# csyxwei/FFWM

Measured on AMD Instinct MI355X. Metric: train img/s (128x128, full FFWM GAN step), higher is better.
Workload: dtype f32; 1 GPU; BASELINE configs[2]: full FFWM train step (netG+netD+flowNetF+flowNetB, all losses, 3x Adam), synthetic MultiPIE-shaped 128x128; batch_per_gpu=8, global_batch=8, parallelism=dp1, grad_buckets=10, bucket_MiB=64

## Files before the change

ffwm_amd/_lib.py:

```python
import ctypes
import os

_HERE = os.path.dirname(os.path.abspath(__file__))
LIB_PATH = os.path.join(_HERE, "lib", "libffwm_hip.so")

F32, F64 = 0, 1
ABI_VERSION = 5

_lib = None

_p = ctypes.c_void_p
_i64 = ctypes.c_int64
_i = ctypes.c_int

_SIGNATURES = {
    "ffwm_block_extractor_forward": [_p, _p, _p] + [_i64] * 6 + [_i, _i, _p],
    "ffwm_block_extractor_backward": [_p, _p, _p, _p, _p] + [_i64] * 6 + [_i, _i, _p],
    "ffwm_block_extractor_backward_strided": [_p, _p, _p, ctypes.POINTER(_i64), _p, _p] + [_i64] * 6 + [_i, _i, _p],
    "ffwm_local_attn_reshape_backward_strided": [_p, ctypes.POINTER(_i64), _p] + [_i64] * 3 + [_i, _i, _i, _p],
    "ffwm_resample2d_backward_strided": [_p, _p, _p, ctypes.POINTER(_i64), _p, _p] + [_i64] * 6 + [_i, _i, _i, _i, _p],
    "ffwm_bn_lrelu_forward": [_p] * 9 + [_i64] * 3 + [ctypes.c_double] * 3 + [_i, _p],
    "ffwm_bn_lrelu_backward": [_p] * 10 + [_i64] * 3 + [ctypes.c_double] + [_i, _p],
    "ffwm_bn_res_act_forward": [_p] * 11 + [_i64] * 3 + [ctypes.c_double] * 3 + [_i, _i, _p],
    "ffwm_bn_res_act_backward": [_p] * 11 + [_i64] * 3 + [ctypes.c_double] + [_i, _i, _p],
# ... 23 lines not shown
    "ffwm_sgd_step": [_p, _p, _p, _i64, _p, _p, _i, _p, _p, _i, ctypes.c_double, _i, _p],
    "ffwm_softmax_xent": [_p] * 8 + [_i64, _i64, _i, _p],
    "ffwm_softmax_xent_chunk": [],
    "ffwm_conv3x3_wgrad": [_p, _p, _p, _p] + [_i64] * 5 + [_i, _p],
    "ffwm_conv3x3_wgrad_block": [_p, _p, _p, _p] + [_i64] * 9 + [_i, _p],
    "ffwm_block_attention_forward": [_p, _p, _p, _p] + [_i64] * 6 + [_i, _i, _p],
    "ffwm_block_attention_backward": [_p, _p, _p, _p, _p, _p, _p] + [_i64] * 6 + [_i, _i, _p],
    "ffwm_local_attn_reshape_forward": [_p, _p] + [_i64] * 3 + [_i, _i, _p],
    "ffwm_local_attn_reshape_backward": [_p, _p] + [_i64] * 3 + [_i, _i, _i, _p],
    "ffwm_resample2d_forward": [_p, _p, _p] + [_i64] * 6 + [_i, _i, _i, _p],
    "ffwm_resample2d_backward": [_p, _p, _p, _p, _p] + [_i64] * 6 + [_i, _i, _i, _i, _p],
    "ffwm_warp_forward": [_p, _p, _p] + [_i64] * 6 + [_i, _i, _p],
    "ffwm_warp_backward": [_p, _p, _p, _p, _p] + [_i64] * 6 + [_i, _i, _p],
    "ffwm_warp_multi_forward": [_p, _i, _i, _i, _p],
    "ffwm_warp_multi_backward": [_p, _i, _i, _i, _p],
    "ffwm_spectral_norm_forward": [_p, _i, _i, ctypes.c_double, _i, _p],
    "ffwm_spectral_norm_backward": [_p, _i, _i, _p],
    "ffwm_guided_filter_forward": [_p, _p, _p, _p, _i64, _i64, _i64, _i, ctypes.c_double, _i, _p],
    "ffwm_affine_regularization": [_p, _p, _p, _p, _i64, _i64, _i64, _i, ctypes.c_double, _i, _p],
    "ffwm_correlation_colmax": [_p, _p, _p, _i64, _i64, _i64, _i, _p],
    "ffwm_correlation_colmax_split": [_p, _p, _p, _i64, _i64, _i64, _i, _p],
    "ffwm_sampling_correctness": [_p] * 9 + [_i64] * 6 + [ctypes.c_double, ctypes.c_double, _i, _p],
    "ffwm_landmark_loss": [_p, _p, ctypes.POINTER(_i64), ctypes.POINTER(_i64), ctypes.POINTER(ctypes.c_double), _i] + [_p] * 6
                          + [_i64, _i64, _i, _p],
    "ffwm_guided_filter_backward": [_p, _p, _p, _p, _p, _p, _i64, _i64, _i64, _i, _i, _p],
    "ffwm_guided_filter_forward_general": [_p, _p, _p, _p, _p, _i64, _i64, _i64, _i64, _i, ctypes.c_double, _i, _p],
    "ffwm_guided_filter_backward_general": [_p, _p, _p, _p, _p, _p, _p, _i64, _i64, _i64, _i64, _i, _i, _p],
    "ffwm_l1_multi": [_p, _i, _p, _p, _i, _i, _p],
    "ffwm_conv3x3_winograd_weights_multi": [_p, _i, _i, _p],
    "ffwm_conv3x3_wg_weights": [_p, _p, _i64, _i64, _i, _i, _p],
    "ffwm_conv3x3_wg_forward": [_p, _p, _p, _p, _p] + [_i64] * 5 + [_i, _p, _i, _p],
    "ffwm_conv3x3_wg_forward_tiled": [_p, _p, _p, _p, _p] + [_i64] * 5 + [_i, _p, _i, _i, _p],
    "ffwm_conv3x3_wg_tile": [_i64] * 5,
    "ffwm_mfm_tail_forward": [_p, _p, _p, _p] + [_i64] * 4 + [_i, _i, _p],
    "ffwm_identity_input": [_p, _p] + [_i64] * 4 + [_i, _i, _p],
    "ffwm_identity_input_backward": [_p, _p] + [_i64] * 4 + [_i, _i, _p],
    "ffwm_cosine_topk": [_p, _p, _p, _p] + [_i64] * 4 + [_p, _i64, _i, _p],
    "ffwm_face_batch": [_p] * 16 + [_i64] * 8 + [_i, _p],
    "ffwm_face_gallery": [_p, _p, _p] + [_i64] * 4 + [_p],
    "ffwm_identity_batch": [_p] * 8 + [_i64] * 5 + [_i, _i, _p],
    "ffwm_prof_enable": [_i],
    "ffwm_prof_collect": [],
    "ffwm_prof_get": [_i, ctypes.c_char_p, _i, ctypes.POINTER(_i64), ctypes.POINTER(ctypes.c_double),
                      ctypes.POINTER(ctypes.c_double)],
    "ffwm_prof_get_flops": [_i, ctypes.POINTER(ctypes.c_double)],
    "ffwm_prof_get_bound": [_i, ctypes.POINTER(ctypes.c_double)],
    "ffwm_prof_reset": [],
    "ffwm_set_option": [ctypes.c_char_p, _i],
    "ffwm_zero_fill": [_p, _i64, _p],
    "ffwm_abi_version": [],
}

EXPORTS = sorted(list(_SIGNATURES) + ["ffwm_last_error", "ffwm_conv3x3_winograd_workspace_bytes", "ffwm_conv3x3_winograd_splits",
                                      "ffwm_conv2d_forward_workspace", "ffwm_guided_filter_workspace_bytes",
                                      "ffwm_sampling_correctness_workspace_bytes", "ffwm_landmark_loss_workspace_bytes",
                                      "ffwm_cosine_topk_workspace_bytes", "ffwm_softmax_xent_workspace_bytes",
                                      "ffwm_conv3x3_wg_weights_bytes", "ffwm_conv3x3_wg_workspace_bytes"])


class FFWMError(RuntimeError):
    pass


def load():
    global _lib
    if _lib is not None:
        return _lib
    if not os.path.exists(LIB_PATH):
        raise FFWMError(
            "libffwm_hip.so is missing (%s). The HIP extension is the only implementation of the "
            "ffwm_amd ops -- build it with `python -m ffwm_amd.build`." % LIB_PATH)
    lib = ctypes.CDLL(LIB_PATH)
    for name, argtypes in _SIGNATURES.items():
        fn = getattr(lib, name)
        fn.argtypes = argtypes
        fn.restype = _i
    lib.ffwm_conv3x3_winograd_workspace_bytes.argtypes = [_i64, _i64]
    lib.ffwm_conv3x3_winograd_workspace_bytes.restype = _i64
    lib.ffwm_conv3x3_winograd_splits.argtypes = [_i64, _i64, _i64, _i64, _i64, _i]
    lib.ffwm_conv3x3_winograd_splits.restype = _i
    lib.ffwm_conv2d_forward_workspace.argtypes = [_i64] * 5 + [_i] * 4
    lib.ffwm_conv2d_forward_workspace.restype = _i64
    lib.ffwm_guided_filter_workspace_bytes.argtypes = [_i64] * 4 + [_i, _i]
    lib.ffwm_guided_filter_workspace_bytes.restype = _i64
    lib.ffwm_sampling_correctness_workspace_bytes.argtypes = [_i64, _i64, _i64, _i]
    lib.ffwm_sampling_correctness_workspace_bytes.restype = _i64
    lib.ffwm_landmark_loss_workspace_bytes.argtypes = [ctypes.POINTER(_i64), _i, _i64, _i64, _i]
    lib.ffwm_landmark_loss_workspace_bytes.restype = _i64
    lib.ffwm_softmax_xent_workspace_bytes.argtypes = [_i64, _i64, _i]
    lib.ffwm_softmax_xent_workspace_bytes.restype = _i64
    lib.ffwm_cosine_topk_workspace_bytes.argtypes = [_i64] * 4
    lib.ffwm_cosine_topk_workspace_bytes.restype = _i64
    lib.ffwm_conv3x3_wg_weights_bytes.argtypes = [_i64, _i64]
    lib.ffwm_conv3x3_wg_weights_bytes.restype = _i64
    lib.ffwm_conv3x3_wg_workspace_bytes.argtypes = [_i64] * 5
    lib.ffwm_conv3x3_wg_workspace_bytes.restype = _i64
    lib.ffwm_last_error.argtypes = []
    lib.ffwm_last_error.restype = ctypes.c_char_p
    got = lib.ffwm_abi_version()
    if got != ABI_VERSION:
        raise FFWMError("libffwm_hip.so ABI version %d, expected %d: rebuild it" % (got, ABI_VERSION))
    _lib = lib
    for kv in filter(None, os.environ.get("FFWM_OPTS", "").split(",")):
        k, _, v = kv.partition("=")
        if lib.ffwm_set_option(k.strip().encode(), int(v)) < 0:
            raise FFWMError("FFWM_OPTS: unknown option %r (or a negative value)" % k)
    return lib


def check(rc, what):
    if rc != 0:
        msg = load().ffwm_last_error()
        raise FFWMError("%s failed (status %d): %s" % (what, rc, msg.decode() if msg else "?"))


def prof_enable(on=True):
    return load().ffwm_prof_enable(1 if on else 0)


def prof_reset():
    load().ffwm_prof_reset()


def prof_collect():
    lib = load()
    n = lib.ffwm_prof_collect()
    rows = {}
    for i in range(n):
        name = ctypes.create_string_buffer(128)
# ... 22 lines not shown
```

ffwm_amd/conv.py:

```python
import os as _os

import torch
import torch.nn as nn
from torch.autograd import Function

from . import ops

_WGRAD_W64 = _os.environ.get("FFWM_WGRAD_W64", "1") == "1"


class _Conv3x3MfmaWgrad(Function):

    @staticmethod
    def forward(ctx, x, weight, bias):
        ctx.save_for_backward(x, weight)
        ctx.has_bias = bias is not None
        return torch.ops.aten.convolution(x, weight, bias, [1, 1], [1, 1], [1, 1], False, [0, 0], 1)

    @staticmethod
    @torch.autograd.function.once_differentiable
    def backward(ctx, grad_output):
        x, weight = ctx.saved_tensors
        go = grad_output.contiguous()
        need_x, need_w, need_b = ctx.needs_input_grad[0], ctx.needs_input_grad[1], ctx.has_bias and ctx.needs_input_grad[2]
# ... 77 lines not shown
        self.off = self.need = 0
        if self.buf is not None and self.buf.device != device:
            self.retired.append(self.buf)
            self.buf = None
        if self.buf is not None:
            ops.zero_fill(self.buf)
        self.active = True
        self.device = device

    def take(self, n, like):
        if not self.active or like.device != self.device or like.dtype != torch.float32:
            return None
        n_al = (n + 63) & ~63
        self.need += n_al
        if self.buf is None or self.off + n_al > self.buf.numel():
            return None
        s = self.buf[self.off:self.off + n]
        self.off += n_al
        return s

    def end(self):
        if not self.active:
            return
        self.active = False
        if (self.buf is None or self.need > self.buf.numel()) and self.need > 0 and not torch.cuda.is_current_stream_capturing():
            if self.buf is not None:
                self.retired.append(self.buf)
            self.buf = torch.zeros(self.need + self.need // 8, device=self.device, dtype=torch.float32)


GRAD_ARENA = _GradArena()


def conv_weight_grad(x, go, weight, stride, pad, need_b):
    k = weight.shape[2]
    if k == 3 and stride == 1 and pad == 1 and wgrad_route_ok(x, weight):
        n = weight.numel()
        total = n + (weight.shape[0] if need_b else 0)
        buf = GRAD_ARENA.take(total, go)
        if buf is None:
            buf = torch.zeros(total, device=go.device, dtype=go.dtype)
        gw, gb = buf[:n].view_as(weight), (buf[n:] if need_b else None)
        ops.conv3x3_wgrad(x, go, gw, gb)
        return gw, gb
    if _tiled_wgrad_wins(go, x, k) and weight.shape[2] == weight.shape[3]:
        return ops.conv2d_wgrad_tiled(go, x, k, stride, pad, want_bias=bool(need_b),
                                      zeroed=GRAD_ARENA.take(weight.numel() + (weight.shape[0] if need_b else 0), go))
    _, gw, gb = torch.ops.aten.convolution_backward(go, x, weight, [weight.shape[0]] if need_b else None, [stride, stride], [pad, pad],
                                                    [1, 1], False, [0, 0], 1, [False, True, bool(need_b)])
    return gw, gb


def conv_transpose_weight_grad(x, go, weight, need_b):
    if _tiled_wgrad_wins(x, go, 4):
        gw, _ = ops.conv2d_wgrad_tiled(x, go, 4, 2, 1, zeroed=GRAD_ARENA.take(weight.numel(), go))
        return gw, (_bias_grad(go) if need_b else None)
    _, gw, gb = torch.ops.aten.convolution_backward(go, x, weight, [weight.shape[1]] if need_b else None, [2, 2], [1, 1], [1, 1], True,
                                                    [0, 0], 1, [False, True, bool(need_b)])
    return gw, gb


_WINOGRAD = _os.environ.get("FFWM_WINOGRAD", "1") != "0"
WINOGRAD_MIN_TILES = int(_os.environ.get("FFWM_WINOGRAD_MIN_TILES", 2048))
WINOGRAD_MIN_PAIRS = int(_os.environ.get("FFWM_WINOGRAD_MIN_PAIRS", 160))


def _winograd_dir_ok(x, c_red, k_out, act=0):
    tiles = x.shape[0] * ((x.shape[2] + 1) // 2) * ((x.shape[3] + 1) // 2)
    if not (min(c_red, k_out) >= 32 and tiles >= WINOGRAD_MIN_TILES and x.shape[0] * max(c_red, k_out) * x.shape[2] * x.shape[3] < (1 << 29)):
        return False
    pairs = ((tiles + 63) // 64) * ((k_out + 63) // 64)
    if pairs < WINOGRAD_MIN_PAIRS and act == 0:
        pairs *= ops.conv3x3_winograd_splits(x.shape[0], c_red, x.shape[2], x.shape[3], k_out, act)
    return pairs >= WINOGRAD_MIN_PAIRS


def winograd_dirs(x, weight, act=0):
# ... 544 lines not shown
```

ffwm_amd/csrc/conv_winograd_gemm.hip:

```cpp
#include "common.hpp"

namespace ffwm {
namespace {

typedef float f32x16 __attribute__((ext_vector_type(16)));
typedef float f32x4 __attribute__((ext_vector_type(4)));

enum { kWgNone = FFWM_WG_NONE, kWgBias = FFWM_WG_BIAS, kWgBiasRelu = FFWM_WG_BIAS_RELU, kWgBiasMfm = FFWM_WG_BIAS_MFM };
constexpr int kWgStage = 16;

struct WgGeo {
    int C, C4;
    int H, W, K;
    int TH, TW, T;
    int Tp, Kp;
};

__device__ __forceinline__ float wg_max_nan(float a, float b) { return __builtin_isunordered(a, b) ? a + b : fmaxf(a, b); }
__device__ __forceinline__ float wg_relu_nan(float v) { return v != v ? v : fmaxf(v, 0.f); }

__global__ void __launch_bounds__(kBlock)
wg_weights_kernel(const float* __restrict__ w, float* __restrict__ U, int K, int C, int Cp, int mode) {
    const int64_t e = static_cast<int64_t>(blockIdx.x) * kBlock + threadIdx.x;
    if (e >= static_cast<int64_t>(K) * Cp) return;
// ... 49 lines not shown
        for (int i = 0; i < 4; ++i)
#pragma unroll
            for (int q = 0; q < 4; ++q) {
                const int iy = 2 * ty - 1 + i, ix = 2 * tx - 1 + q;
                float e = 0.f;
                if (cv && iy >= 0 && iy < g.H && ix >= 0 && ix < g.W) {
                    const size_t o = plane + static_cast<size_t>(iy) * g.W + ix;
                    e = x[o];
                    if (mask != nullptr) e = mask[o] <= 0.f ? 0.f : e;
                }
                d[i * 4 + q] = e;
            }
#pragma unroll
        for (int i = 0; i < 4; ++i) {
            float r[4];
#pragma unroll
            for (int q = 0; q < 4; ++q)
                r[q] = i == 0 ? d[0 + q] - d[8 + q] : i == 1 ? d[4 + q] + d[8 + q] : i == 2 ? d[8 + q] - d[4 + q] : d[4 + q] - d[12 + q];
            v[i * 4 + 0][j] = r[0] - r[2];
            v[i * 4 + 1][j] = r[1] + r[2];
            v[i * 4 + 2][j] = r[2] - r[1];
            v[i * 4 + 3][j] = r[1] - r[3];
        }
    }
    const size_t pstride = static_cast<size_t>(g.C4) * g.Tp;
    f32x4* dst = reinterpret_cast<f32x4*>(V) + static_cast<size_t>(c4) * g.Tp + t;
#pragma unroll
    for (int p = 0; p < 16; ++p) dst[p * pstride] = v[p];
}

template <int TILE>
__global__ void __launch_bounds__(kBlock)
wg_batched_gemm_kernel(const float* __restrict__ U, const float* __restrict__ V, float* __restrict__ M, int K, int C4, int Tp, int Kp,
                       int KT, int TTn) {
    constexpr int WT = TILE / 2, NB = WT / 32, NL = TILE / 64;
    __shared__ f32x4 As[2][4][TILE];
    __shared__ f32x4 Bs[2][4][TILE];
    const int lane = threadIdx.x & 63, wave = threadIdx.x >> 6;
    const int l31 = lane & 31, half = lane >> 5;
    const int wm = wave >> 1, wn = wave & 1;
    unsigned bid = blockIdx.x;
    const int tt = static_cast<int>(bid % static_cast<unsigned>(TTn));
    bid /= static_cast<unsigned>(TTn);
    const int kt = static_cast<int>(bid % static_cast<unsigned>(KT));
    const int p = static_cast<int>(bid / static_cast<unsigned>(KT));
    const int k0 = kt * TILE, t0 = tt * TILE;
    const f32x4* Up = reinterpret_cast<const f32x4*>(U) + static_cast<size_t>(p) * C4 * K;
    const f32x4* Vp = reinterpret_cast<const f32x4*>(V) + static_cast<size_t>(p) * C4 * Tp;

    f32x4 ra[NL], rb[NL];
    auto gload = [&](int stage) {
#pragma unroll
        for (int i = 0; i < NL; ++i) {
            const int idx = threadIdx.x + kBlock * i;
            const int grp = stage * 4 + idx / TILE, n = idx % TILE;
            f32x4 a = {0.f, 0.f, 0.f, 0.f};
            if (k0 + n < K) a = Up[static_cast<size_t>(grp) * K + k0 + n];
            ra[i] = a;
            rb[i] = Vp[static_cast<size_t>(grp) * Tp + t0 + n];
        }
    };
    auto sstore = [&](int buf) {
#pragma unroll
        for (int i = 0; i < NL; ++i) {
            const int idx = threadIdx.x + kBlock * i;
            As[buf][idx / TILE][idx % TILE] = ra[i];
            Bs[buf][idx / TILE][idx % TILE] = rb[i];
        }
    };

    f32x16 acc[NB][NB];
#pragma unroll
    for (int i = 0; i < NB; ++i)
#pragma unroll
        for (int j = 0; j < NB; ++j)
#pragma unroll
            for (int r = 0; r < 16; ++r) acc[i][j][r] = 0.f;

    const int stages = C4 / 4;
    gload(0);
    sstore(0);
    __syncthreads();
    int buf = 0;
    for (int st = 0; st < stages; ++st) {
        const bool more = st + 1 < stages;
        if (more) gload(st + 1);
#pragma unroll
        for (int s = 0; s < 2; ++s) {
            f32x4 a[NB], b[NB];
#pragma unroll
            for (int i = 0; i < NB; ++i) {
                a[i] = As[buf][2 * s + half][wm * WT + i * 32 + l31];
                b[i] = Bs[buf][2 * s + half][wn * WT + i * 32 + l31];
            }
#pragma unroll
            for (int q = 0; q < 4; ++q)
#pragma unroll
                for (int i = 0; i < NB; ++i)
#pragma unroll
                    for (int j = 0; j < NB; ++j)
                        acc[i][j] = __builtin_amdgcn_mfma_f32_32x32x2f32(a[i][q], b[j][q], acc[i][j], 0, 0, 0);
        }
        if (more) sstore(buf ^ 1);
        __syncthreads();
        buf ^= 1;
    }

    float* Mp = M + (static_cast<size_t>(p) * Kp + k0 + wm * WT) * Tp + t0 + wn * WT + l31;
#pragma unroll
    for (int i = 0; i < NB; ++i)
#pragma unroll
        for (int j = 0; j < NB; ++j)
#pragma unroll
            for (int r = 0; r < 16; ++r) {
                const int row = i * 32 + (r & 3) + 8 * (r >> 2) + 4 * half;
                Mp[static_cast<size_t>(row) * Tp + j * 32] = acc[i][j][r];
            }
}

__device__ __forceinline__ void wg_tile_of(const float* __restrict__ M, size_t pstride, float bv, float (&y)[4]) {
    float z[4][2];
#pragma unroll
    for (int i = 0; i < 4; ++i) {
        const float m0 = M[(i * 4 + 0) * pstride], m1 = M[(i * 4 + 1) * pstride], m2 = M[(i * 4 + 2) * pstride], m3 = M[(i * 4 + 3) * pstride];
        z[i][0] = (m0 + m1) + m2;
        z[i][1] = (m1 - m2) - m3;
    }
#pragma unroll
    for (int j = 0; j < 2; ++j) {
        y[j] = ((z[0][j] + z[1][j]) + z[2][j]) + bv;
        y[2 + j] = ((z[1][j] - z[2][j]) - z[3][j]) + bv;
    }
}

__global__ void __launch_bounds__(kBlock)
wg_output_transform_kernel(const float* __restrict__ M, const float* __restrict__ bias, float* __restrict__ out, const WgGeo g, int epi,
                           int vec) {
    const int t = blockIdx.x * kBlock + threadIdx.x;
    if (t >= g.T) return;
    const int ko = blockIdx.y;
    const int Kout = epi == kWgBiasMfm ? g.K / 2 : g.K;
    const size_t pstride = static_cast<size_t>(g.Kp) * g.Tp;
    const bool use_bias = bias != nullptr && epi != kWgNone;
    float y[4];
    wg_tile_of(M + static_cast<size_t>(ko) * g.Tp + t, pstride, use_bias ? bias[ko] : 0.f, y);
    if (epi == kWgBiasRelu) {
#pragma unroll
        for (int v = 0; v < 4; ++v) y[v] = wg_relu_nan(y[v]);
    } else if (epi == kWgBiasMfm) {
        float y2[4];
        wg_tile_of(M + static_cast<size_t>(ko + Kout) * g.Tp + t, pstride, use_bias ? bias[ko + Kout] : 0.f, y2);
#pragma unroll
        for (int v = 0; v < 4; ++v) y[v] = wg_max_nan(y[v], y2[v]);
    }
    const int per = g.TH * g.TW;
    const int b = t / per, rem = t - b * per;
    const int ty = rem / g.TW, tx = rem - ty * g.TW;
    const int oy = 2 * ty, ox = 2 * tx;
    const bool row1 = oy + 1 < g.H, col1 = ox + 1 < g.W;
    float* o = out + ((static_cast<size_t>(b) * Kout + ko) * g.H + oy) * g.W + ox;
    if (vec) {
        *reinterpret_cast<float2*>(o) = make_float2(y[0], y[1]);
        if (row1) *reinterpret_cast<float2*>(o + g.W) = make_float2(y[2], y[3]);
    } else {
        o[0] = y[0];
        if (col1) o[1] = y[1];
        if (row1) {
            o[g.W] = y[2];
            if (col1) o[g.W + 1] = y[3];
        }
    }
}

}
}

using namespace ffwm;

static int64_t wg_round_up(int64_t v, int64_t m) { return (v + m - 1) / m * m; }

struct WgPlan {
    int tile;
    int64_t T, Tp, Kp, Cp;
    int64_t KT, TTn;
    int64_t v_floats, m_floats;
};
static WgPlan wg_plan(int64_t B, int64_t C, int64_t H, int64_t W, int64_t K, int force_tile) {
    WgPlan p;
    p.T = B * ((H + 1) / 2) * ((W + 1) / 2);
    p.Cp = wg_round_up(C, kWgStage);
    const int64_t n128 = 16 * ((K + 127) / 128) * ((p.T + 127) / 128);
    p.tile = force_tile ? force_tile : (n128 >= device_cus() ? 128 : 64);
    p.Tp = wg_round_up(p.T, p.tile);
    p.Kp = wg_round_up(K, p.tile);
    p.KT = p.Kp / p.tile;
    p.TTn = p.Tp / p.tile;
    p.v_floats = 16 * p.Cp * p.Tp;
    p.m_floats = 16 * p.Kp * p.Tp;
    return p;
}

extern "C" int64_t ffwm_conv3x3_wg_weights_bytes(int64_t K, int64_t C) {
// ... 44 lines not shown
    const int epi = epilogue;
    FFWM_REQUIRE(epi >= kWgNone && epi <= kWgBiasMfm, FFWM_ERR_ARG,
                 "%s: epilogue must be 0 (none), 1 (bias), 2 (bias, relu) or 3 (bias, max-feature-map)", fn);
    FFWM_REQUIRE(tile == 0 || tile == 64 || tile == 128, FFWM_ERR_ARG, "%s: tile must be 0 (the plan's), 64 or 128", fn);
    FFWM_REQUIRE(epi != kWgBiasMfm || K % 2 == 0, FFWM_ERR_ARG, "%s: the max-feature-map epilogue needs an even K", fn);
    FFWM_REQUIRE(reinterpret_cast<uintptr_t>(workspace) % 16 == 0 && reinterpret_cast<uintptr_t>(U) % 16 == 0, FFWM_ERR_ARG,
                 "%s: U and the workspace must be 16-byte aligned", fn);
    FFWM_REQUIRE(B * C * H * W < (1LL << 31) && B * K * H * W < (1LL << 31), FFWM_ERR_SIZE, "%s: a tensor beyond 2^31 elements", fn);
    const WgPlan p = wg_plan(B, C, H, W, K, tile);
    const int64_t Kout = epi == kWgBiasMfm ? K / 2 : K;
    FFWM_REQUIRE(p.Tp < (1LL << 30) && p.Cp / 4 <= 65535 && Kout <= 65535 && 16 * p.KT * p.TTn < (1LL << 31), FFWM_ERR_SIZE,
                 "%s: too many tiles or channels", fn);
    WgGeo g;
    g.C = static_cast<int>(C); g.C4 = static_cast<int>(p.Cp / 4);
    g.H = static_cast<int>(H); g.W = static_cast<int>(W); g.K = static_cast<int>(K);
    g.TH = static_cast<int>((H + 1) / 2); g.TW = static_cast<int>((W + 1) / 2); g.T = static_cast<int>(p.T);
    g.Tp = static_cast<int>(p.Tp); g.Kp = static_cast<int>(p.Kp);
    hipStream_t st = static_cast<hipStream_t>(stream);
    float* V = static_cast<float*>(workspace);
    float* M = V + p.v_floats;
    const double act = static_cast<double>(B) * H * W;
    {
        LaunchScope ls("conv_wg_in", st, 4.0 * (act * C * (relu_mask ? 2.0 : 1.0) + static_cast<double>(p.v_floats)));
        hipLaunchKernelGGL(wg_input_transform_kernel, dim3(static_cast<unsigned>((p.Tp + kBlock - 1) / kBlock), static_cast<unsigned>(g.C4)),
                           dim3(kBlock), 0, st, static_cast<const float*>(input), static_cast<const float*>(relu_mask), V, g);
    }
    if (int rc = check_launch(fn)) return rc;
    {
        LaunchScope ls("conv_wg_gemm", st, 4.0 * (16.0 * K * p.Cp + static_cast<double>(p.v_floats) + static_cast<double>(p.m_floats)),
                       2.0 * 16.0 * static_cast<double>(p.T) * K * C);
        const unsigned grid = static_cast<unsigned>(16 * p.KT * p.TTn);
        const bool ok = dispatch<64, 128>(p.tile, [&](auto TILE) {
            hipLaunchKernelGGL(wg_batched_gemm_kernel<TILE.value>, dim3(grid), dim3(kBlock), 0, st, static_cast<const float*>(U), V, M, g.K,
                               g.C4, g.Tp, g.Kp, static_cast<int>(p.KT), static_cast<int>(p.TTn));
        });
        if (!ok) return no_kernel(fn);
    }
    if (int rc = check_launch(fn)) return rc;
    {
        LaunchScope ls("conv_wg_out", st, 4.0 * (16.0 * K * p.T + act * Kout));
        const int vec = W % 2 == 0 && reinterpret_cast<uintptr_t>(output) % 8 == 0;
        hipLaunchKernelGGL(wg_output_transform_kernel, dim3(static_cast<unsigned>((p.T + kBlock - 1) / kBlock), static_cast<unsigned>(Kout)),
                           dim3(kBlock), 0, st, M, static_cast<const float*>(bias), static_cast<float*>(output), g, epi, vec);
    }
    return check_launch(fn);
}
```

ffwm_amd/ops.py:

```python
import ctypes

import torch

from . import _lib

_DT = {torch.float32: _lib.F32, torch.float64: _lib.F64}


def _dtype_code(t):
    try:
        return _DT[t.dtype]
    except KeyError:
        raise TypeError("ffwm_amd ops support float32/float64 (AT_DISPATCH_FLOATING_TYPES), got %s" % t.dtype)


def _go_strides(grad_output):
    if grad_output.is_contiguous():
        return grad_output, None
    st = grad_output.stride()
    if any(x < 0 for x in st) or st[3] == 0:
        return grad_output.contiguous(), None
    return grad_output, (ctypes.c_int64 * 4)(*st)


# ... 759 lines not shown
    if x.dtype != torch.float32:
        raise TypeError("conv3x3_wg: float32 only")
    B, C, H, W = x.shape
    if K is None:
        if bias is None:
            raise ValueError("conv3x3_wg: K is needed when there is no bias")
        K = bias.numel()
    lib = _lib.load()
    if U.numel() * 4 != lib.ffwm_conv3x3_wg_weights_bytes(K, C):
        raise ValueError("conv3x3_wg: U does not belong to a layer with %d input and %d output channels" % (C, K))
    if bias is not None and (not bias.is_contiguous() or bias.numel() != K):
        raise ValueError("conv3x3_wg: bias must be a contiguous vector of %d elements" % K)
    if relu_mask is not None and (relu_mask.shape != x.shape or not relu_mask.is_contiguous()):
        raise ValueError("conv3x3_wg: relu_mask must be contiguous and of x's shape")
    epi = WG_EPILOGUES[epilogue]
    if epi == 3 and K % 2:
        raise ValueError("conv3x3_wg: the mfm epilogue needs an even K")
    shape = (B, K // 2 if epi == 3 else K, H, W)
    if out is None:
        out = x.new_empty(shape)
    elif tuple(out.shape) != shape:
        raise ValueError("conv3x3_wg: out has the wrong shape")
    ws = x.new_empty((lib.ffwm_conv3x3_wg_workspace_bytes(B, C, H, W, K) // 4,))
    with _on_device(x) as stream:
        _lib.check(lib.ffwm_conv3x3_wg_forward_tiled(_ptr(x), _ptr(U), _ptr(bias), _ptr(out), _ptr(ws), B, C, H, W, K, epi,
                                                     _ptr(relu_mask), int(tile), _dtype_code(x), stream), "ffwm_conv3x3_wg_forward")
    return out


def conv3x3_wg_tile(B, C, H, W, K):
    return int(_lib.load().ffwm_conv3x3_wg_tile(int(B), int(C), int(H), int(W), int(K)))


def _mfm_dims(x):
    if x.dim() < 2 or x.shape[1] % 2:
        raise ValueError("mfm: need [B, 2C, ...], got %s" % (tuple(x.shape),))
    hw = 1
    for d in x.shape[2:]:
        hw *= d
    return x.shape[0], x.shape[1] // 2, hw


def _bias_ok(x, bias, n):
    if bias is None:
        return
    if not (bias.is_cuda and bias.dtype == x.dtype and bias.is_contiguous() and bias.numel() == n):
        raise ValueError("bias must be a contiguous float32 GPU vector of %d elements" % n)


_ACT_CODES = {"lrelu": 1, "sigmoid": 3}


def _same_f32(name, *ts):
    t0 = ts[0]
    for t in ts:
        if not (t.is_cuda and t.dtype == torch.float32 and t.is_contiguous() and t.shape == t0.shape and t.device == t0.device):
            raise NotImplementedError("%s: contiguous float32 GPU tensors of one shape only" % name)


def add_act_forward(a, b, act, negative_slope=0.2):
    _same_f32("add_act_forward", a, b)
    y = torch.empty_like(a)
    if y.numel():
        with _on_device(a) as stream:
            _lib.check(_lib.load().ffwm_add_act_forward(_ptr(a), _ptr(b), _ptr(y), a.numel(), _ACT_CODES[act], float(negative_slope),
                                                        _lib.F32, stream), "ffwm_add_act_forward")
# ... 374 lines not shown
```

include/ffwm_hip.h:

```cpp
#ifndef FFWM_HIP_H_
#define FFWM_HIP_H_

#include <stdint.h>

#ifdef __cplusplus
extern "C" {
#endif

#define FFWM_ABI_VERSION 5

typedef enum {
    FFWM_OK = 0,
    FFWM_ERR_ARG = -1,
    FFWM_ERR_DTYPE = -2,
    FFWM_ERR_SIZE = -3,
    FFWM_ERR_LAUNCH = -4
} ffwm_status;

typedef enum { FFWM_F32 = 0, FFWM_F64 = 1 } ffwm_dtype;

int ffwm_abi_version(void);
const char* ffwm_last_error(void);

int ffwm_block_extractor_forward(const void* source, const void* flow_field, void* output,
// ... 207 lines not shown
                      int64_t C, int64_t H, int64_t W, int kernel, int stride, int pad, int dtype, void* stream);

int ffwm_conv2d_wgrad_tiled(const void* rows, const void* gathered, void* grad_weight, void* grad_bias, int64_t B, int64_t K,
                            int64_t Ho, int64_t Wo, int64_t C, int64_t H, int64_t W, int kernel, int stride, int pad, int prezeroed,
                            int dtype, void* stream);

int64_t ffwm_conv3x3_winograd_workspace_bytes(int64_t K, int64_t C);
int ffwm_conv3x3_winograd_splits(int64_t B, int64_t C, int64_t H, int64_t W, int64_t K, int act);

typedef struct ffwm_wino_weights {
    const void* weight;
    void* workspace;
    int64_t K, C;
    int data_gradient;
    int width_multiple_of_4;
} ffwm_wino_weights;
int ffwm_conv3x3_winograd_weights_multi(const ffwm_wino_weights* items, int n, int dtype, void* stream);
int ffwm_conv3x3_winograd_forward(const void* input, const void* weight, const void* bias, void* output, void* workspace,
                                  int64_t B, int64_t C, int64_t H, int64_t W, int64_t K, int data_gradient, int act,
                                  double slope, int dtype, void* stream);

enum { FFWM_WG_NONE = 0, FFWM_WG_BIAS = 1, FFWM_WG_BIAS_RELU = 2, FFWM_WG_BIAS_MFM = 3 };
int64_t ffwm_conv3x3_wg_weights_bytes(int64_t K, int64_t C);
int64_t ffwm_conv3x3_wg_workspace_bytes(int64_t B, int64_t C, int64_t H, int64_t W, int64_t K);
int ffwm_conv3x3_wg_weights(const void* weight, void* U, int64_t K, int64_t C, int data_gradient, int dtype, void* stream);
int ffwm_conv3x3_wg_forward(const void* input, const void* U, const void* bias, void* output, void* workspace,
                            int64_t B, int64_t C, int64_t H, int64_t W, int64_t K, int epilogue, const void* relu_mask,
                            int dtype, void* stream);
int ffwm_conv3x3_wg_tile(int64_t B, int64_t C, int64_t H, int64_t W, int64_t K);
int ffwm_conv3x3_wg_forward_tiled(const void* input, const void* U, const void* bias, void* output, void* workspace,
                                  int64_t B, int64_t C, int64_t H, int64_t W, int64_t K, int epilogue, const void* relu_mask,
                                  int tile, int dtype, void* stream);

int ffwm_adam_step(void* params, const void* grads, void* exp_avg, void* exp_avg_sq, int64_t n, double lr,
                   double beta1, double beta2, double eps, int64_t step, int dtype, void* stream);

int ffwm_adam_step_device(void* params, const void* grads, void* exp_avg, void* exp_avg_sq, int64_t n, double lr, double beta1,
                          double beta2, double eps, void* state, int dtype, void* stream);

int ffwm_sgd_step(void* params, const void* grads, void* momentum_buf, int64_t n, const int64_t* seg_end, const int32_t* seg_group,
                  int n_seg, const double* group_lr, const double* group_wd, int n_groups, double momentum, int dtype, void* stream);

int ffwm_softmax_xent_chunk(void);
int64_t ffwm_softmax_xent_workspace_bytes(int64_t B, int64_t N, int dtype);
int ffwm_softmax_xent(const void* logits, const int64_t* target, void* out, void* row_loss, int* rank, void* grad_logits,
                      int* skipped, void* workspace, int64_t B, int64_t N, int dtype, void* stream);

int ffwm_shuffle_bias_act_forward(const void* h, const void* bias, void* y, int64_t B, int64_t K, int64_t H, int64_t W,
                                  int64_t y_batch_stride, double negative_slope, int dtype, void* stream);
int ffwm_image_head_forward(const void* x, const void* weight, const void* bias, void* y, int64_t B, int64_t C, int64_t H, int64_t W,
                            int64_t y_batch_stride, int dtype, void* stream);
int ffwm_upsample2x_bilinear_forward(const void* x, void* y, int64_t B, int64_t C, int64_t H, int64_t W, int64_t y_batch_stride,
                                     int dtype, void* stream);
int ffwm_sigmoid_gate_forward_strided(const void* a, const void* b, const void* x, void* att, void* y, int64_t B, int64_t C,
                                      int64_t HW, int64_t y_batch_stride, int dtype, void* stream);

int ffwm_mfm_tail_forward(const void* h, const void* bias, const void* residual, void* y, int64_t B, int64_t C, int64_t H, int64_t W,
                          int pool, int dtype, void* stream);
int ffwm_identity_input(const void* img, void* out, int64_t B, int64_t Cin, int64_t H, int64_t W, int crop, int dtype, void* stream);
int ffwm_identity_input_backward(const void* grad_out, void* grad_img, int64_t B, int64_t Cin, int64_t H, int64_t W, int crop, int dtype,
                                 void* stream);
int64_t ffwm_cosine_topk_workspace_bytes(int64_t B, int64_t G, int64_t D, int64_t k);
int ffwm_cosine_topk(const void* probe, const void* gallery, void* values, void* indices, int64_t B, int64_t G, int64_t D, int64_t k,
                     void* workspace, int64_t workspace_bytes, int dtype, void* stream);

int ffwm_face_batch(const void* images, const void* masks, const void* pairs, const void* pair_lm, const void* lm, const void* lm_flip,
// ... 25 lines not shown
```

Measured before the change: 222.8 img/s.

## Add Winograd F(2x2,3x3) weight-gradient path for mid-size 3x3 convolutions

Adds a Winograd-domain weight-gradient route for 3x3 stride-1 convolutions. It transforms the input and grad_output into 16 Winograd planes, runs a batched GEMM that reuses the forward kernel with split-K slots over tile groups, then reduces the slots, inverse-transforms to 3x3 taps and sums bias partials. The route applies only to channel/tile-count combinations listed in a table, replacing the tiled direct wgrad for those layers. It adds workspace allocation per call and may differ slightly numerically from the direct reduction.

```diff
diff --git a/ffwm_amd/_lib.py b/ffwm_amd/_lib.py
--- a/ffwm_amd/_lib.py
+++ b/ffwm_amd/_lib.py
@@ -79,6 +79,8 @@
     "ffwm_conv3x3_wg_forward": [_p, _p, _p, _p, _p] + [_i64] * 5 + [_i, _p, _i, _p],
     "ffwm_conv3x3_wg_forward_tiled": [_p, _p, _p, _p, _p] + [_i64] * 5 + [_i, _p, _i, _i, _p],
     "ffwm_conv3x3_wg_tile": [_i64] * 5,
+    "ffwm_conv3x3_wgrad_wg_plan": [_i64] * 5 + [_i, _i, ctypes.POINTER(_i64)],
+    "ffwm_conv3x3_wgrad_wg": [_p] * 5 + [_i64] * 5 + [_i, _i, _i, _p],
     "ffwm_mfm_tail_forward": [_p, _p, _p, _p] + [_i64] * 4 + [_i, _i, _p],
     "ffwm_identity_input": [_p, _p] + [_i64] * 4 + [_i, _i, _p],
     "ffwm_identity_input_backward": [_p, _p] + [_i64] * 4 + [_i, _i, _p],
@@ -102,7 +104,8 @@
                                       "ffwm_conv2d_forward_workspace", "ffwm_guided_filter_workspace_bytes",
                                       "ffwm_sampling_correctness_workspace_bytes", "ffwm_landmark_loss_workspace_bytes",
                                       "ffwm_cosine_topk_workspace_bytes", "ffwm_softmax_xent_workspace_bytes",
-                                      "ffwm_conv3x3_wg_weights_bytes", "ffwm_conv3x3_wg_workspace_bytes"])
+                                      "ffwm_conv3x3_wg_weights_bytes", "ffwm_conv3x3_wg_workspace_bytes",
+                                      "ffwm_conv3x3_wgrad_wg_workspace_bytes"])
 
 
 class FFWMError(RuntimeError):
@@ -142,6 +145,8 @@
     lib.ffwm_conv3x3_wg_weights_bytes.restype = _i64
     lib.ffwm_conv3x3_wg_workspace_bytes.argtypes = [_i64] * 5
     lib.ffwm_conv3x3_wg_workspace_bytes.restype = _i64
+    lib.ffwm_conv3x3_wgrad_wg_workspace_bytes.argtypes = [_i64] * 5
+    lib.ffwm_conv3x3_wgrad_wg_workspace_bytes.restype = _i64
     lib.ffwm_last_error.argtypes = []
     lib.ffwm_last_error.restype = ctypes.c_char_p
     got = lib.ffwm_abi_version()
diff --git a/ffwm_amd/conv.py b/ffwm_amd/conv.py
--- a/ffwm_amd/conv.py
+++ b/ffwm_amd/conv.py
@@ -133,6 +133,25 @@
 GRAD_ARENA = _GradArena()
 
 
+_WGW = _os.environ.get("FFWM_WGRAD_GEMM", "1") != "0"
+
+WGW_TABLE = {
+    (384, 384): (2048, 2048),
+    (384, 256): (2048, 2048),
+    (256, 256): (512, 2048),
+    (256, 512): (512, 512),
+    (512, 512): (128, 128),
+}
+
+
+def wgrad_gemm_ok(x, go, weight):
+    if not (_WGW and x.is_cuda and x.dtype == torch.float32 and go.dtype == torch.float32 and x.dim() == 4
+            and x.shape[2] % 2 == 0 and x.shape[3] % 2 == 0 and not torch.is_autocast_enabled()):
+        return False
+    rng = WGW_TABLE.get((weight.shape[1], weight.shape[0]))
+    return rng is not None and rng[0] <= x.shape[0] * (x.shape[2] // 2) * (x.shape[3] // 2) <= rng[1]
+
+
 def conv_weight_grad(x, go, weight, stride, pad, need_b):
     k = weight.shape[2]
     if k == 3 and stride == 1 and pad == 1 and wgrad_route_ok(x, weight):
@@ -144,6 +163,8 @@
         gw, gb = buf[:n].view_as(weight), (buf[n:] if need_b else None)
         ops.conv3x3_wgrad(x, go, gw, gb)
         return gw, gb
+    if k == 3 and stride == 1 and pad == 1 and weight.shape[3] == 3 and wgrad_gemm_ok(x, go, weight):
+        return ops.conv3x3_wgrad_wg(x, go, want_bias=bool(need_b))
     if _tiled_wgrad_wins(go, x, k) and weight.shape[2] == weight.shape[3]:
         return ops.conv2d_wgrad_tiled(go, x, k, stride, pad, want_bias=bool(need_b),
                                       zeroed=GRAD_ARENA.take(weight.numel() + (weight.shape[0] if need_b else 0), go))
diff --git a/ffwm_amd/csrc/conv_winograd_gemm.hip b/ffwm_amd/csrc/conv_winograd_gemm.hip
--- a/ffwm_amd/csrc/conv_winograd_gemm.hip
+++ b/ffwm_amd/csrc/conv_winograd_gemm.hip
@@ -105,7 +105,7 @@
 template <int TILE>
 __global__ void __launch_bounds__(kBlock)
 wg_batched_gemm_kernel(const float* __restrict__ U, const float* __restrict__ V, float* __restrict__ M, int K, int C4, int Tp, int Kp,
-                       int KT, int TTn) {
+                       int KT, int TTn, int G, size_t m_slot) {
     constexpr int WT = TILE / 2, NB = WT / 32, NL = TILE / 64;
     __shared__ f32x4 As[2][4][TILE];
     __shared__ f32x4 Bs[2][4][TILE];
@@ -116,8 +116,9 @@
     const int tt = static_cast<int>(bid % static_cast<unsigned>(TTn));
     bid /= static_cast<unsigned>(TTn);
     const int kt = static_cast<int>(bid % static_cast<unsigned>(KT));
-    const int p = static_cast<int>(bid / static_cast<unsigned>(KT));
-    const int k0 = kt * TILE, t0 = tt * TILE;
+    bid /= static_cast<unsigned>(KT);
+    const int p = static_cast<int>(bid & 15u), slot = static_cast<int>(bid >> 4);
+    const int k0 = kt * TILE, t0 = tt * TILE, g0 = slot * G;
     const f32x4* Up = reinterpret_cast<const f32x4*>(U) + static_cast<size_t>(p) * C4 * K;
     const f32x4* Vp = reinterpret_cast<const f32x4*>(V) + static_cast<size_t>(p) * C4 * Tp;
 
@@ -126,7 +127,7 @@
 #pragma unroll
         for (int i = 0; i < NL; ++i) {
             const int idx = threadIdx.x + kBlock * i;
-            const int grp = stage * 4 + idx / TILE, n = idx % TILE;
+            const int grp = g0 + stage * 4 + idx / TILE, n = idx % TILE;
             f32x4 a = {0.f, 0.f, 0.f, 0.f};
             if (k0 + n < K) a = Up[static_cast<size_t>(grp) * K + k0 + n];
             ra[i] = a;
@@ -150,7 +151,7 @@
 #pragma unroll
             for (int r = 0; r < 16; ++r) acc[i][j][r] = 0.f;
 
-    const int stages = C4 / 4;
+    const int stages = G / 4;
     gload(0);
     sstore(0);
     __syncthreads();
@@ -179,7 +180,7 @@
         buf ^= 1;
     }
 
-    float* Mp = M + (static_cast<size_t>(p) * Kp + k0 + wm * WT) * Tp + t0 + wn * WT + l31;
+    float* Mp = M + static_cast<size_t>(slot) * m_slot + (static_cast<size_t>(p) * Kp + k0 + wm * WT) * Tp + t0 + wn * WT + l31;
 #pragma unroll
     for (int i = 0; i < NB; ++i)
 #pragma unroll
@@ -241,6 +242,140 @@
         if (row1) {
             o[g.W] = y[2];
             if (col1) o[g.W + 1] = y[3];
+        }
+    }
+}
+
+constexpr unsigned kWgwOob = 0xFFFFFFF0u;
+
+struct WgwGeo {
+    int N;
+    int rows;
+    int H, W, TH, TW, T, Tq;
+    unsigned bytes;
+};
+
+template <bool DY>
+__global__ void __launch_bounds__(kBlock)
+wgw_transform_kernel(const float* __restrict__ src, float* __restrict__ dst, float* __restrict__ bias_part, const WgwGeo g) {
+    const int tql = (threadIdx.x & 3) + 4 * (threadIdx.x >> 6), cl = (threadIdx.x >> 2) & 15;
+    const int tq = blockIdx.x * 16 + tql, ch = blockIdx.y * 16 + cl;
+    const bool ch_ok = ch < g.N;
+    const rsrc_t rs = make_rsrc(src, g.bytes);
+    const int per = g.TH * g.TW;
+    const unsigned w4 = static_cast<unsigned>(g.W) * 4u;
+    f32x4 v[16];
+    float bsum = 0.f;
+#pragma unroll
+    for (int j = 0; j < 4; ++j) {
+        const int t = tq * 4 + j;
+        const bool live = ch_ok && t < g.T;
+        const int ts = live ? t : 0;
+        const int b = ts / per, rem = ts - b * per;
+        const int ty = rem / g.TW, tx = rem - ty * g.TW;
+        const unsigned o = (((static_cast<unsigned>(b) * g.N + (live ? ch : 0)) * g.H + 2 * ty) * g.W + 2 * tx) * 4u;
+        if constexpr (DY) {
+            const u32x2 r0 = __builtin_amdgcn_raw_buffer_load_b64(rs, live ? o : kWgwOob, 0, 0);
+            const u32x2 r1 = __builtin_amdgcn_raw_buffer_load_b64(rs, live ? o + w4 : kWgwOob, 0, 0);
+            const float a = __uint_as_float(r0.x), bb = __uint_as_float(r0.y), c = __uint_as_float(r1.x), d = __uint_as_float(r1.y);
+            bsum += (a + bb) + (c + d);
+            const float rp[4] = {a, a + c, a - c, -c}, rq[4] = {bb, bb + d, bb - d, -d};
+#pragma unroll
+            for (int i = 0; i < 4; ++i) {
+                v[i * 4 + 0][j] = rp[i];
+                v[i * 4 + 1][j] = rp[i] + rq[i];
+                v[i * 4 + 2][j] = rp[i] - rq[i];
+                v[i * 4 + 3][j] = -rq[i];
+            }
+        } else {
+            float d[16];
+#pragma unroll
+            for (int i = 0; i < 4; ++i) {
+                const int iy = 2 * ty - 1 + i;
+                const bool rok = live && iy >= 0 && iy < g.H;
+                const unsigned orow = o + static_cast<unsigned>(i - 1) * w4;
+                const u32x2 m = __builtin_amdgcn_raw_buffer_load_b64(rs, rok ? orow : kWgwOob, 0, 0);
+                d[i * 4 + 0] = __uint_as_float(__builtin_amdgcn_raw_buffer_load_b32(rs, (rok && tx > 0) ? orow - 4u : kWgwOob, 0, 0));
+                d[i * 4 + 1] = __uint_as_float(m.x);
+                d[i * 4 + 2] = __uint_as_float(m.y);
+                d[i * 4 + 3] = __uint_as_float(__builtin_amdgcn_raw_buffer_load_b32(rs, (rok && tx + 1 < g.TW) ? orow + 8u : kWgwOob, 0, 0));
+            }
+#pragma unroll
+            for (int i = 0; i < 4; ++i) {
+                float r[4];
+#pragma unroll
+                for (int q = 0; q < 4; ++q)
+                    r[q] = i == 0 ? d[0 + q] - d[8 + q] : i == 1 ? d[4 + q] + d[8 + q] : i == 2 ? d[8 + q] - d[4 + q] : d[4 + q] - d[12 + q];
+                v[i * 4 + 0][j] = r[0] - r[2];
+                v[i * 4 + 1][j] = r[1] + r[2];
+                v[i * 4 + 2][j] = r[2] - r[1];
+                v[i * 4 + 3][j] = r[1] - r[3];
+            }
+        }
+    }
+    if (tq < g.Tq && ch < g.rows) {
+        const size_t pstride = static_cast<size_t>(g.Tq) * g.rows;
+        f32x4* out = reinterpret_cast<f32x4*>(dst) + static_cast<size_t>(tq) * g.rows + ch;
+#pragma unroll
+        for (int p = 0; p < 16; ++p) out[p * pstride] = v[p];
+    }
+    if constexpr (DY) {
+        __shared__ float sb[4][16];
+        float s = bsum;
+        s += __shfl_xor(s, 1, 64);
+        s += __shfl_xor(s, 2, 64);
+        if ((threadIdx.x & 3) == 0) sb[threadIdx.x >> 6][cl] = s;
+        __syncthreads();
+        if (threadIdx.x < 16 && blockIdx.y * 16 + threadIdx.x < g.N)
+            bias_part[static_cast<size_t>(blockIdx.x) * g.N + blockIdx.y * 16 + threadIdx.x] =
+                ((sb[0][threadIdx.x] + sb[1][threadIdx.x]) + sb[2][threadIdx.x]) + sb[3][threadIdx.x];
+    }
+}
+
+__global__ void __launch_bounds__(kBlock)
+wgw_epilogue_kernel(const float* __restrict__ dU, const float* __restrict__ bias_part, float* __restrict__ dW, float* __restrict__ dbias,
+                    int K, int C, int Kp, int Cp, int slots, int bias_blocks) {
+    __shared__ __attribute__((aligned(16))) float taps[kBlock * 9];
+    const int e0 = blockIdx.x * kBlock, e = e0 + threadIdx.x;
+    if (dbias != nullptr && e < K) {
+        float s = bias_part[e];
+        for (int blk = 1; blk < bias_blocks; ++blk) s += bias_part[static_cast<size_t>(blk) * K + e];
+        dbias[e] = s;
+    }
+    if (e < K * C) {
+        const int k = e / C, c = e - k * C;
+        const size_t pstride = static_cast<size_t>(Kp) * Cp, sstride = 16 * pstride;
+        const float* src = dU + static_cast<size_t>(k) * Cp + c;
+        float u[16];
+#pragma unroll
+        for (int p = 0; p < 16; ++p) u[p] = src[p * pstride];
+        for (int s = 1; s < slots; ++s)
+#pragma unroll
+            for (int p = 0; p < 16; ++p) u[p] += src[s * sstride + p * pstride];
+        float z[4][3];
+#pragma unroll
+        for (int i = 0; i < 4; ++i) {
+            const float u0 = u[i * 4 + 0], u1 = u[i * 4 + 1], u2 = u[i * 4 + 2], u3 = u[i * 4 + 3];
+            z[i][0] = u0 + 0.5f * (u1 + u2);
+            z[i][1] = 0.5f * (u1 - u2);
+            z[i][2] = 0.5f * (u1 + u2) + u3;
+        }
+        float* o = taps + threadIdx.x * 9;
+#pragma unroll
+        for (int s = 0; s < 3; ++s) {
+            o[0 + s] = z[0][s] + 0.5f * (z[1][s] + z[2][s]);
+            o[3 + s] = 0.5f * (z[1][s] - z[2][s]);
+            o[6 + s] = 0.5f * (z[1][s] + z[2][s]) + z[3][s];
+        }
+    }
+    __syncthreads();
+    const int n = min(kBlock, K * C - e0) * 9;
+    float* dst = dW + static_cast<size_t>(e0) * 9;
+    for (int i = threadIdx.x * 4; i < n; i += kBlock * 4) {
+        if (i + 4 <= n) {
+            *reinterpret_cast<f32x4*>(dst + i) = *reinterpret_cast<const f32x4*>(taps + i);
+        } else {
+            for (int j = i; j < n; ++j) dst[j] = taps[j];
         }
     }
 }
@@ -351,7 +486,7 @@
         const unsigned grid = static_cast<unsigned>(16 * p.KT * p.TTn);
         const bool ok = dispatch<64, 128>(p.tile, [&](auto TILE) {
             hipLaunchKernelGGL(wg_batched_gemm_kernel<TILE.value>, dim3(grid), dim3(kBlock), 0, st, static_cast<const float*>(U), V, M, g.K,
-                               g.C4, g.Tp, g.Kp, static_cast<int>(p.KT), static_cast<int>(p.TTn));
+                               g.C4, g.Tp, g.Kp, static_cast<int>(p.KT), static_cast<int>(p.TTn), g.C4, static_cast<size_t>(0));
         });
         if (!ok) return no_kernel(fn);
     }
@@ -364,3 +499,124 @@
     }
     return check_launch(fn);
 }
+
+struct WgwPlan {
+    int tile;
+    int64_t T, Tq;
+    int64_t Kp, Cp, KT, CTn;
+    int64_t slots, groups;
+    int64_t bias_blocks;
+    int64_t v_floats, dm_floats, du_floats, bias_floats;
+    int64_t floats() const { return v_floats + dm_floats + du_floats + bias_floats; }
+};
+static WgwPlan wgw_plan(int64_t B, int64_t C, int64_t K, int64_t H, int64_t W, int force_tile, int force_slots) {
+    WgwPlan p;
+    p.T = B * (H / 2) * (W / 2);
+    const int64_t stages = (p.T + kWgStage - 1) / kWgStage;
+    p.tile = force_tile ? force_tile : 64;
+    p.Kp = wg_round_up(K, p.tile);
+    p.Cp = wg_round_up(C, p.tile);
+    p.KT = p.Kp / p.tile;
+    p.CTn = p.Cp / p.tile;
+    int64_t slots = force_slots;
+    if (slots <= 0) {
+        const int64_t wgs = 16 * p.KT * p.CTn;
+        slots = (4 * device_cus() + wgs - 1) / wgs;
+        if (slots > stages / 4) slots = stages / 4;
+        if (slots > 8) slots = 8;
+    }
+    if (slots > stages) slots = stages;
+    if (slots < 1) slots = 1;
+    const int64_t per = (stages + slots - 1) / slots;
+    p.slots = (stages + per - 1) / per;
+    p.groups = 4 * per;
+    p.Tq = p.slots * p.groups;
+    p.bias_blocks = (p.Tq + 15) / 16;
+    p.v_floats = 16 * p.Tq * p.Cp * 4;
+    p.dm_floats = 16 * p.Tq * K * 4;
+    p.du_floats = p.slots * 16 * p.Kp * p.Cp;
+    p.bias_floats = p.bias_blocks * K;
+    return p;
+}
+
+static bool wgw_shape_ok(int64_t B, int64_t C, int64_t K, int64_t H, int64_t W) {
+    return B > 0 && C > 0 && K > 0 && H > 0 && W > 0 && H % 2 == 0 && W % 2 == 0;
+}
+
+extern "C" int64_t ffwm_conv3x3_wgrad_wg_workspace_bytes(int64_t B, int64_t C, int64_t K, int64_t H, int64_t W) {
+    if (!wgw_shape_ok(B, C, K, H, W)) return 0;
+    return wgw_plan(B, C, K, H, W, 0, 0).floats() * 4;
+}
+
+extern "C" int ffwm_conv3x3_wgrad_wg_plan(int64_t B, int64_t C, int64_t K, int64_t H, int64_t W, int tile, int slots, int64_t* out) {
+    const char* fn = "ffwm_conv3x3_wgrad_wg_plan";
+    FFWM_REQUIRE(out, FFWM_ERR_ARG, "%s: NULL result pointer", fn);
+    FFWM_REQUIRE(wgw_shape_ok(B, C, K, H, W), FFWM_ERR_ARG, "%s: sizes must be positive, H and W even", fn);
+    FFWM_REQUIRE(tile == 0 || tile == 64 || tile == 128, FFWM_ERR_ARG, "%s: tile must be 0 (the plan's), 64 or 128", fn);
+    FFWM_REQUIRE(slots >= 0, FFWM_ERR_ARG, "%s: slots must be 0 (the plan's) or positive", fn);
+    const WgwPlan p = wgw_plan(B, C, K, H, W, tile, slots);
+    out[0] = p.tile; out[1] = p.slots; out[2] = p.groups; out[3] = p.Tq;
+    out[4] = p.Kp; out[5] = p.Cp; out[6] = p.bias_blocks; out[7] = p.floats() * 4;
+    return FFWM_OK;
+}
+
+extern "C" int ffwm_conv3x3_wgrad_wg(const void* input, const void* grad_output, void* grad_weight, void* grad_bias, void* workspace,
+                                     int64_t B, int64_t C, int64_t K, int64_t H, int64_t W, int tile, int slots, int dtype, void* stream) {
+    const char* fn = "ffwm_conv3x3_wgrad_wg";
+    FFWM_REQUIRE(dtype == FFWM_F32, FFWM_ERR_DTYPE, "%s: float32 only", fn);
+    FFWM_REQUIRE(input && grad_output && grad_weight && workspace, FFWM_ERR_ARG, "%s: NULL tensor pointer", fn);
+    FFWM_REQUIRE(wgw_shape_ok(B, C, K, H, W), FFWM_ERR_ARG, "%s: sizes must be positive, H and W even", fn);
+    FFWM_REQUIRE(tile == 0 || tile == 64 || tile == 128, FFWM_ERR_ARG, "%s: tile must be 0 (the plan's), 64 or 128", fn);
+    FFWM_REQUIRE(slots >= 0, FFWM_ERR_ARG, "%s: slots must be 0 (the plan's) or positive", fn);
+    FFWM_REQUIRE(reinterpret_cast<uintptr_t>(workspace) % 16 == 0 && reinterpret_cast<uintptr_t>(grad_weight) % 16 == 0, FFWM_ERR_ARG,
+                 "%s: the workspace and grad_weight must be 16-byte aligned", fn);
+    FFWM_REQUIRE(reinterpret_cast<uintptr_t>(input) % 8 == 0 && reinterpret_cast<uintptr_t>(grad_output) % 8 == 0, FFWM_ERR_ARG,
+                 "%s: input and grad_output must be 8-byte aligned", fn);
+    FFWM_REQUIRE(B * C * H * W < (1LL << 29) && B * K * H * W < (1LL << 29) && K * C * 9 < (1LL << 29), FFWM_ERR_SIZE,
+                 "%s: a tensor beyond 2 GiB", fn);
+    const WgwPlan p = wgw_plan(B, C, K, H, W, tile, slots);
+    FFWM_REQUIRE(p.v_floats < (1LL << 29) && p.dm_floats < (1LL << 29) && p.du_floats < (1LL << 29), FFWM_ERR_SIZE,
+                 "%s: a transformed operand beyond 2 GiB", fn);
+    FFWM_REQUIRE(p.Cp / 16 <= 65535 && (K + 15) / 16 <= 65535 && p.slots * 16 * p.KT * p.CTn < (1LL << 31), FFWM_ERR_SIZE,
+                 "%s: too many tiles or channels", fn);
+    hipStream_t st = static_cast<hipStream_t>(stream);
+    float* V = static_cast<float*>(workspace);
+    float* dM = V + p.v_floats;
+    float* dU = dM + p.dm_floats;
+    float* bias_part = dU + p.du_floats;
+    const double act = static_cast<double>(B) * H * W;
+    WgwGeo g;
+    g.H = static_cast<int>(H); g.W = static_cast<int>(W); g.TH = static_cast<int>(H / 2); g.TW = static_cast<int>(W / 2);
+    g.T = static_cast<int>(p.T); g.Tq = static_cast<int>(p.Tq);
+    {
+        LaunchScope ls("conv_wgw_transform", st, 4.0 * (act * (C + K) + static_cast<double>(p.v_floats + p.dm_floats)));
+        const unsigned gx = static_cast<unsigned>(p.bias_blocks);
+        g.N = static_cast<int>(C); g.rows = static_cast<int>(p.Cp); g.bytes = static_cast<unsigned>(B * C * H * W * 4);
+        hipLaunchKernelGGL(wgw_transform_kernel<false>, dim3(gx, static_cast<unsigned>(p.Cp / 16)), dim3(kBlock), 0, st,
+                           static_cast<const float*>(input), V, static_cast<float*>(nullptr), g);
+        g.N = static_cast<int>(K); g.rows = static_cast<int>(K); g.bytes = static_cast<unsigned>(B * K * H * W * 4);
+        hipLaunchKernelGGL(wgw_transform_kernel<true>, dim3(gx, static_cast<unsigned>((K + 15) / 16)), dim3(kBlock), 0, st,
+                           static_cast<const float*>(grad_output), dM, bias_part, g);
+    }
+    if (int rc = check_launch(fn)) return rc;
+    {
+        LaunchScope ls("conv_wgw_gemm", st, 4.0 * static_cast<double>(p.v_floats + p.dm_floats + p.du_floats),
+                       2.0 * 16.0 * static_cast<double>(p.T) * K * C);
+        const unsigned grid = static_cast<unsigned>(p.slots * 16 * p.KT * p.CTn);
+        const bool ok = dispatch<64, 128>(p.tile, [&](auto TILE) {
+            hipLaunchKernelGGL(wg_batched_gemm_kernel<TILE.value>, dim3(grid), dim3(kBlock), 0, st, dM, V, dU, static_cast<int>(K),
+                               static_cast<int>(p.Tq), static_cast<int>(p.Cp), static_cast<int>(p.Kp), static_cast<int>(p.KT),
+                               static_cast<int>(p.CTn), static_cast<int>(p.groups), static_cast<size_t>(16 * p.Kp * p.Cp));
+        });
+        if (!ok) return no_kernel(fn);
+    }
+    if (int rc = check_launch(fn)) return rc;
+    {
+        LaunchScope ls("conv_wgw_epilogue", st, 4.0 * (static_cast<double>(p.slots) * 16.0 * K * C + 9.0 * K * C + static_cast<double>(p.bias_floats)));
+        hipLaunchKernelGGL(wgw_epilogue_kernel, dim3(static_cast<unsigned>((K * C + kBlock - 1) / kBlock)), dim3(kBlock), 0, st, dU,
+                           bias_part, static_cast<float*>(grad_weight), static_cast<float*>(grad_bias), static_cast<int>(K),
+                           static_cast<int>(C), static_cast<int>(p.Kp), static_cast<int>(p.Cp), static_cast<int>(p.slots),
+                           static_cast<int>(p.bias_blocks));
+    }
+    return check_launch(fn);
+}
diff --git a/ffwm_amd/ops.py b/ffwm_amd/ops.py
--- a/ffwm_amd/ops.py
+++ b/ffwm_amd/ops.py
@@ -815,6 +815,39 @@
     return int(_lib.load().ffwm_conv3x3_wg_tile(int(B), int(C), int(H), int(W), int(K)))
 
 
+WGW_PLAN_FIELDS = ("tile", "slots", "groups", "Tq", "Kp", "Cp", "bias_blocks", "workspace_bytes")
+
+
+def conv3x3_wgrad_wg_plan(B, C, K, H, W, tile=0, slots=0):
+    import ctypes
+    out = (ctypes.c_int64 * len(WGW_PLAN_FIELDS))()
+    _lib.check(_lib.load().ffwm_conv3x3_wgrad_wg_plan(int(B), int(C), int(K), int(H), int(W), int(tile), int(slots), out),
+               "ffwm_conv3x3_wgrad_wg_plan")
+    return dict(zip(WGW_PLAN_FIELDS, (int(v) for v in out)))
+
+
+def conv3x3_wgrad_wg(x, go, want_bias=False, tile=0, slots=0):
+    _check("conv3x3_wgrad_wg", x, go)
+    if x.dtype != torch.float32:
+        raise TypeError("conv3x3_wgrad_wg: float32 only")
+    B, C, H, W = x.shape
+    K = go.shape[1]
+    if go.shape[0] != B or tuple(go.shape[2:]) != (H, W):
+        raise ValueError("conv3x3_wgrad_wg: grad_output must be [B, K, H, W] of the input's batch and plane")
+    if H % 2 or W % 2:
+        raise ValueError("conv3x3_wgrad_wg: even H and W only")
+    lib = _lib.load()
+    nbytes = (conv3x3_wgrad_wg_plan(B, C, K, H, W, tile, slots)["workspace_bytes"] if (tile or slots)
+              else lib.ffwm_conv3x3_wgrad_wg_workspace_bytes(B, C, K, H, W))
+    ws = x.new_empty((nbytes // 4,))
+    gw = x.new_empty((K, C, 3, 3))
+    gb = x.new_empty((K,)) if want_bias else None
+    with _on_device(x) as stream:
+        _lib.check(lib.ffwm_conv3x3_wgrad_wg(_ptr(x), _ptr(go), _ptr(gw), _ptr(gb), _ptr(ws), B, C, K, H, W, int(tile), int(slots),
+                                             _dtype_code(x), stream), "ffwm_conv3x3_wgrad_wg")
+    return gw, gb
+
+
 def _mfm_dims(x):
     if x.dim() < 2 or x.shape[1] % 2:
         raise ValueError("mfm: need [B, 2C, ...], got %s" % (tuple(x.shape),))
diff --git a/include/ffwm_hip.h b/include/ffwm_hip.h
--- a/include/ffwm_hip.h
+++ b/include/ffwm_hip.h
@@ -263,6 +263,11 @@
                                   int64_t B, int64_t C, int64_t H, int64_t W, int64_t K, int epilogue, const void* relu_mask,
                                   int tile, int dtype, void* stream);
 
+int64_t ffwm_conv3x3_wgrad_wg_workspace_bytes(int64_t B, int64_t C, int64_t K, int64_t H, int64_t W);
+int ffwm_conv3x3_wgrad_wg_plan(int64_t B, int64_t C, int64_t K, int64_t H, int64_t W, int tile, int slots, int64_t* out);
+int ffwm_conv3x3_wgrad_wg(const void* input, const void* grad_output, void* grad_weight, void* grad_bias, void* workspace,
+                          int64_t B, int64_t C, int64_t K, int64_t H, int64_t W, int tile, int slots, int dtype, void* stream);
+
 int ffwm_adam_step(void* params, const void* grads, void* exp_avg, void* exp_avg_sq, int64_t n, double lr,
                    double beta1, double beta2, double eps, int64_t step, int dtype, void* stream);
 
```

Result: no change. 225.9 img/s, median of 6 (+1.4%).
